# Chanuk-Yang/Deep_Continuous_Fusion_for_Multi-Sensor_3D_Object_Detection

Hardware: AMD Instinct MI355X
Metric: frames/sec (train step) 100k-pt LiDAR + 1242x375 RGB (higher is better)
Workload: dtype bf16; 1 GPU; cfg2: grid 32x704x800, 100000 pts/frame, 1242x375 RGB, ResNet-18 image stream, K=3 fusion x4 sites, eval-mode BN (reference F4), batch 2/GPU; global_batch=2, parallelism=dp1, loss_sampling=compat, conv_chain=False

## Files before the change

### deep_continuous_fusion_for_multi-sensor_3d_object_detection_amd/csrc/conv_common.h

```cpp
#pragma once
#include "dcf_common.h"

namespace {

typedef __bf16 bf16x8 __attribute__((ext_vector_type(8)));
typedef float f32x16 __attribute__((ext_vector_type(16)));
typedef short s16x4 __attribute__((ext_vector_type(4)));

template <int N> __device__ __forceinline__ void wait_vmcnt() { asm volatile("s_waitcnt vmcnt(%0)" ::"n"(N) : "memory"); }
template <int N> __device__ __forceinline__ void wait_vmcnt_nomem() { asm volatile("s_waitcnt vmcnt(%0)" ::"n"(N)); }

__device__ __forceinline__ void glds16(__amdgpu_buffer_rsrc_t rsrc, unsigned voff, unsigned lds_dst)
{
    unsigned keep;
    asm volatile("s_mov_b32 %0, m0\n\ts_mov_b32 m0, %3\n\ts_nop 0\n\tbuffer_load_dwordx4 %1, %2, 0 offen lds\n\ts_mov_b32 m0, %0"
                 : "=&s"(keep)
                 : "v"(voff), "s"(rsrc), "s"(lds_dst)
                 : "memory");
}
__device__ __forceinline__ unsigned lds_addr(const void *p)
{
    return (unsigned)(uintptr_t)(__attribute__((address_space(3))) const char *)p;
}

template <typename V> __device__ __forceinline__ V opaque(V v) { asm volatile("" : "+v"(v)); return v; }

template <typename T> struct Mma;
template <> struct Mma<bf16_t> {
    __device__ static __forceinline__ void run(const uint4 &a, const uint4 &b, f32x16 &acc)
    {
        acc = __builtin_amdgcn_mfma_f32_32x32x16_bf16(__builtin_bit_cast(bf16x8, a), __builtin_bit_cast(bf16x8, b), acc, 0, 0, 0);
    }
};
typedef _Float16 f16x8 __attribute__((ext_vector_type(8)));
template <> struct Mma<f16_t> {
    __device__ static __forceinline__ void run(const uint4 &a, const uint4 &b, f32x16 &acc)
    {
        acc = __builtin_amdgcn_mfma_f32_32x32x16_f16(__builtin_bit_cast(f16x8, a), __builtin_bit_cast(f16x8, b), acc, 0, 0, 0);
    }
};
template <> struct Mma<float> {
// ... 85 lines not shown
```

### deep_continuous_fusion_for_multi-sensor_3d_object_detection_amd/csrc/conv_rs.hip

```cpp
#include "conv_rs_kernel.h"

int dcf_conv3x3_rs_launch(int dtype, const void *x, const void *w, const float *shift, const void *res, const void *mask, void *y,
                          int B, int H, int W, int Ck, int Cn, int relu, int flip, const char *name_base, double flops, hipStream_t s)
{
    if (dtype == DCF_F32 || Ck % 64 || Cn % 64) return DCF_EUNSUPPORTED;
    const int64_t Q = (int64_t)B * H * (W + 2);
    if (Q >= (1ll << 30) || (int64_t)B * H * W * Ck * 2 >= (1ll << 31) || (int64_t)B * H * W * Cn * 2 >= 0xFFFFFF00ll) return DCF_EUNSUPPORTED;
    const RsPlan p = rs_plan(Q, Cn);
    if (p.kind < 0) return DCF_EUNSUPPORTED;
    RsArgs a;
    a.x = (const char *)x; a.w = (const char *)w; a.shift = shift; a.res = (const char *)res; a.mask = (const char *)mask; a.y = (char *)y;
    a.B = B; a.H = H; a.W = W; a.Ck = Ck; a.Cn = Cn; a.relu = relu; a.flip = flip;
    a.npt = p.npt; a.Q = (int)Q;
    a.dbg = dcf_ablate_opt("RS_DBG");
    a.mtiles = (int)((Q + 32 * p.npt - 1) / (32 * p.npt));
    a.xbytes = (unsigned)((int64_t)B * H * W * Ck * 2);
    a.wbytes = (unsigned)((int64_t)Cn * 9 * Ck * 2);
    a.ybytes = (unsigned)((int64_t)B * H * W * Cn * 2);
    const int BN = RS_KINDS[p.kind].BN;
    static DcfOpt pe_o("RS_PERSIST"); const char *pe = pe_o.str();
    int64_t nwg = (((int64_t)a.mtiles * (Cn / BN) + 7) / 8) * 8;
    if (!(pe && atoi(pe) == 0)) nwg = std::min<int64_t>(nwg, 256 * RS_KINDS[p.kind].per_cu);
    const dim3 grid((unsigned)nwg);
    char name[96];
    static DcfOpt pfn_o("RS_PF"); const char *pfn = pfn_o.str();
    static DcfOpt pfn2_o("RS_PF2"), pfl_o("RS_L16"), pfs_o("RS_S3");
    const bool small_pf = p.kind == 2 && !(pfn && atoi(pfn) == 0) && !(pfn2_o.str() && atoi(pfn2_o.str()) == 0) && !(pfl_o.str() && atoi(pfl_o.str()) == 0) &&
                          !(pfs_o.str() && atoi(pfs_o.str()) == 0);
    const bool one_round_n = (Q + 32 * p.npt - 1) / (32 * p.npt) * (Cn / RS_KINDS[p.kind].BN) <= 256 * RS_KINDS[p.kind].per_cu;
    const bool pf_name = small_pf || (p.kind != 2 && ((pfn && atoi(pfn) == 2) || (!(pfn && atoi(pfn) == 0) && (Ck >= 128 || one_round_n))));
    snprintf(name, sizeof(name), pf_name ? "%s<rs%d,%d,pf>" : "%s<rs%d,%d>", name_base, p.kind, p.npt);
    const double bytes = (double)a.xbytes + (double)a.wbytes + (double)B * H * W * Cn * 2.0 * (1 + (res ? 1 : 0) + (mask ? 1 : 0));
    static DcfOpt s3e_o("RS_S3"); const char *s3e = s3e_o.str();
    const bool s3 = !(s3e && atoi(s3e) == 0);
    static DcfOpt l16_o("RS_L16"); const char *l16e = l16_o.str();
    const bool l16 = !(l16e && atoi(l16e) == 0);
    static DcfOpt dx2_o("RS_DX2"); const char *dx2e = dx2_o.str();
    const bool dx2 = p.kind == 1 && p.npt <= 8 && !(dx2e && atoi(dx2e) == 0);
    static DcfOpt pf_o("RS_PF"); const char *pfe = pf_o.str();
    const bool one_round = (int64_t)a.mtiles * (Cn / RS_KINDS[p.kind].BN) <= 256 * RS_KINDS[p.kind].per_cu;
    const bool pf = (pfe && atoi(pfe) == 2) || (!(pfe && atoi(pfe) == 0) && (Ck >= 128 || one_round));
    static DcfOpt pf2_o("RS_PF2"); const char *pf2e = pf2_o.str();
    const bool pf2 = p.kind == 2 && !(pfe && atoi(pfe) == 0) && !(pf2e && atoi(pf2e) == 0);
#define DCF_RS(T_)                                                                                                               \
    do {                                                                                                                         \
        if (p.kind == 0 && pf) DCF_LAUNCH_WB(name, flops, bytes, s, hipLaunchKernelGGL((k_conv3x3_rs<T_, 1, 5, 4, 2, 2, 1, false, false, 0, true>), grid, dim3(512), 0, s, a)); \
        else if (dx2 && pf) DCF_LAUNCH_WB(name, flops, bytes, s, hipLaunchKernelGGL((k_conv3x3_rs<T_, 1, 2, 2, 4, 2, 2, false, false, 0, true>), grid, dim3(512), 0, s, a)); \
        else if (p.kind == 1 && pf) DCF_LAUNCH_WB(name, flops, bytes, s, hipLaunchKernelGGL((k_conv3x3_rs<T_, 1, 3, 2, 4, 2, 1, false, false, 0, true>), grid, dim3(512), 0, s, a)); \
        else if (p.kind == 0) DCF_LAUNCH_WB(name, flops, bytes, s, hipLaunchKernelGGL((k_conv3x3_rs<T_, 1, 5, 4, 2, 2, 1>), grid, dim3(512), 0, s, a)); \
        else if (dx2) DCF_LAUNCH_WB(name, flops, bytes, s, hipLaunchKernelGGL((k_conv3x3_rs<T_, 1, 2, 2, 4, 2, 2>), grid, dim3(512), 0, s, a)); \
        else if (p.kind == 1) DCF_LAUNCH_WB(name, flops, bytes, s, hipLaunchKernelGGL((k_conv3x3_rs<T_, 1, 3, 2, 4, 2, 1>), grid, dim3(512), 0, s, a)); \
        else if (!s3) DCF_LAUNCH_WB(name, flops, bytes, s, hipLaunchKernelGGL((k_conv3x3_rs<T_, 1, 1, 2, 4, 5, 2>), grid, dim3(512), 0, s, a)); \
        else if (l16 && pf2) DCF_LAUNCH_WB(name, flops, bytes, s, hipLaunchKernelGGL((k_conv3x3_rs<T_, 1, 1, 2, 4, 6, 2, true, false, 8, true>), grid, dim3(1024), 0, s, a)); \
        else if (l16) DCF_LAUNCH_WB(name, flops, bytes, s, hipLaunchKernelGGL((k_conv3x3_rs<T_, 1, 1, 2, 4, 6, 2, true, false, 8>), grid, dim3(1024), 0, s, a)); \
        else DCF_LAUNCH_WB(name, flops, bytes, s, hipLaunchKernelGGL((k_conv3x3_rs<T_, 1, 1, 2, 4, 6, 2, true>), grid, dim3(512), 0, s, a)); \
    } while (0)
#ifdef RS_BF16_ONLY
    if (dtype == DCF_F16) return DCF_EUNSUPPORTED;
    DCF_RS(bf16_t);
#else
    if (dtype == DCF_F16) DCF_RS(f16_t); else DCF_RS(bf16_t);
#endif
#undef DCF_RS
    return DCF_OK;
}


#ifdef RS_WSTAMP
extern "C" int dcf_rs_wstamps_read(void *dst, int *dims)
{
    dims[0] = RS_WS_WGS; dims[1] = 8; dims[2] = 3; dims[3] = 64;
    return hipMemcpyFromSymbol(dst, HIP_SYMBOL(g_rs_wstamps), sizeof(g_rs_wstamps)) == hipSuccess ? 0 : -1;
}
extern "C" int dcf_rs_wstamps_clear()
{
    static unsigned zero[RS_WS_WGS * 8 * 3 * 64];
    return hipMemcpyToSymbol(HIP_SYMBOL(g_rs_wstamps), zero, sizeof(zero)) == hipSuccess ? 0 : -1;
}
#endif
```

### deep_continuous_fusion_for_multi-sensor_3d_object_detection_amd/csrc/conv_rs_kernel.h

```cpp
#pragma once
#include <stddef.h>
#include <stdlib.h>

#include <algorithm>
#include <type_traits>

#include "dcf_common.h"
#include "conv_common.h"

#ifndef DCF_RS_SPREAD
#define DCF_RS_SPREAD 1
#endif

namespace {

struct RsArgs {
    const char *x;
    const char *w;
    const float *shift;
    const char *res;
    const char *mask;
    char *y;
    int B, H, W, Ck, Cn;
    int relu, flip;
// ... 1 lines not shown
    int mtiles;
    int Q;
    unsigned xbytes, wbytes, ybytes;
    int dbg;
};

#ifdef RS_STAMP
#define RS_STAMP_WGS 256
#define RS_STAMP_ITEMS 32
__device__ long long g_rs_stamps[RS_STAMP_WGS][RS_STAMP_ITEMS][10];
#define RS_T(k) do { if constexpr (CHAIN) { if (wid == 0) stamp[k] = __builtin_amdgcn_s_memtime(); } } while (0)
#else
#define RS_T(k) do { } while (0)
#endif
#ifdef RS_WSTAMP
#define RS_WS_WGS 256
__device__ unsigned g_rs_wstamps[RS_WS_WGS][8][3][64];
#define RS_WS(reg, idx) do { if constexpr (!CHAIN) { const unsigned t__ = (unsigned)__builtin_amdgcn_s_memtime(); const int i__ = __builtin_amdgcn_readfirstlane(idx); \
    unsigned k__; asm volatile("s_mov_b32 %1, m0\n\ts_mov_b32 m0, %3\n\ts_nop 0\n\tv_writelane_b32 %0, %2, m0\n\ts_mov_b32 m0, %1" : "+v"(reg), "=&s"(k__) : "s"(t__), "s"(i__)); } } while (0)
#else
#define RS_WS(reg, idx) do { } while (0)
#endif
#define RS_CHAIN_MAX 24
struct RsChainLayer {
    const char *x, *w;
    const float *shift;
    const char *res, *mask;
    char *y;
    int relu, pad_;
};
struct RsChainArgs {
    RsArgs a;
    int nlayers;
    int spin_limit;
    int acquire;
    int pad_;
    int *ws;
    RsChainLayer L[RS_CHAIN_MAX];
};
template <typename P> __device__ __forceinline__ P rs_uniform(P p)
{
    const unsigned long long v = (unsigned long long)p;
    const unsigned lo = __builtin_amdgcn_readfirstlane((unsigned)v), hi = __builtin_amdgcn_readfirstlane((unsigned)(v >> 32));
    return (P)(((unsigned long long)hi << 32) | lo);
}
__device__ __forceinline__ const RsArgs &rs_common(const RsArgs &a) { return a; }
// ... 46 lines not shown
    case 5: wait_vmcnt<5>(); break;
    case 6: wait_vmcnt<6>(); break;
    case 7: wait_vmcnt<7>(); break;
    case 8: wait_vmcnt<8>(); break;
    case 9: wait_vmcnt<9>(); break;
    case 10: wait_vmcnt<10>(); break;
    case 11: wait_vmcnt<11>(); break;
    default: wait_vmcnt<12>(); break;
    }
}

constexpr int rs_allowed(int kj, int dw, int dx, int pww, int pxa, int pxb)
{
    int back = dw;
    if (kj == 0 && 3 * dx - 1 < back) back = 3 * dx - 1;
    int n = 0;
    for (int d = 1; d < back; ++d) {
        const int k = ((kj - d) % 3 + 3) % 3;
        n += pww + (k == 0 ? pxa : (k == 1 ? pxb : 0));
    }
    return n;
}

template <typename T, int TN, int TMMAX, int WN, int WM, int DW, int DX, bool S3 = false, bool CHAIN = false, int NL = 0, bool PF = false>
__global__ void __launch_bounds__((WN * WM + NL) * 64) k_conv3x3_rs(typename std::conditional<CHAIN, RsChainArgs, RsArgs>::type arg)
{
    constexpr bool L16 = NL > 0;
    static_assert(!PF || !CHAIN, "the rotated loop: single-layer launches");
    static_assert(!(PF && S3) || NL > 0, "the rotated loop with stage-granular synchronisation: the consumer + loader form only");
    static_assert(!(L16 && CHAIN) && (NL == 0 || NL == 4 || NL == 8), "loader waves: none, four or eight; no chain mode with them");
    const RsArgs &a = rs_common(arg);
    static_assert(DT<T>::size == 2, "16-bit element types only");
    constexpr int NW = WN * WM;
    constexpr int BN = WN * TN * 32;
    constexpr int BMMAX = WM * TMMAX * 32;
    constexpr int NWD = NL ? NL : NW;
    constexpr int PWW = BN / 8 / NWD;
    static_assert(PWW >= 1 && PWW * 8 * NWD == BN, "weight tile must split evenly over the issuing waves");
    constexpr int PXW = (BMMAX + 2 + 8 * NWD - 1) / (8 * NWD);
    constexpr int XROWS = NWD * PXW * 8;
    constexpr int WSLOT = BN * 128, XSLOT = XROWS * 128;
    constexpr int NSW = S3 ? DW + 3 : DW + 1, NSX = DX + 1;
    static_assert(DW >= 1 && DX >= 1 && (DW - 1) * PWW + 2 * PXW <= 48, "vmcnt range");
    static_assert(!S3 || DW == 3 * DX, "stage-granular sync: weights and pixels run the same number of stages ahead");
    static_assert(NSW * WSLOT + NSX * XSLOT <= 160 * 1024, "LDS");
    __shared__ __attribute__((aligned(1024))) char lds[NSW * WSLOT + NSX * XSLOT];

    const int tid = threadIdx.x, lane = tid & 63;
    const int wid16 = __builtin_amdgcn_readfirstlane(tid >> 6);
    const bool loader = L16 && wid16 >= WN * WM;
    const int wid = L16 ? (wid16 >= WN * WM ? wid16 - WN * WM : wid16) : wid16;
    const int wn = wid / WM;
    const int wm = (wid & 4) ? WM - 1 - wid % WM : wid % WM;
    const int r = lane & 31, h = lane >> 5;

    const int nt = a.Cn / BN;
    const int nblk = a.mtiles * nt;
    const int chunk = (nblk + 7) >> 3;
    const int wpx = gridDim.x >> 3;
    const int chunk_lo = (blockIdx.x & 7) * chunk, chunk_hi = min(chunk_lo + chunk, nblk);
    const int gidx_first = chunk_lo + (blockIdx.x >> 3);
    int gidx = gidx_first;
    auto chain_finish = [&]() __attribute__((always_inline)) {
        if constexpr (CHAIN) {
            __builtin_amdgcn_s_barrier();
            int *flag = reinterpret_cast<int *>(lds);
            if (tid == 0) *flag = __hip_atomic_fetch_add(arg.ws, 1, __ATOMIC_RELAXED, __HIP_MEMORY_SCOPE_AGENT) == (int)gridDim.x - 1;
            __syncthreads();
            if (*flag) {
// ... 36 lines not shown
            const kconst_t kp = (kconst_t)__builtin_amdgcn_kernarg_segment_ptr() + offsetof(RsChainArgs, L) +
                                (size_t)__builtin_amdgcn_readfirstlane(l) * sizeof(RsChainLayer);
            const __attribute__((address_space(4))) unsigned long long *q = (const __attribute__((address_space(4))) unsigned long long *)kp;
            static_assert(sizeof(RsChainLayer) == 56 && offsetof(RsChainLayer, y) == 40 && offsetof(RsChainLayer, relu) == 48, "layout read word by word");
            px = (const char *)q[0]; pw = (const char *)q[1]; lshift = (const float *)q[2]; pr = (const char *)q[3]; pm = (const char *)q[4];
            py = (char *)q[5]; lrelu = (int)(unsigned)q[6];
        } else {
            px = a.x; pw = a.w; pr = a.res; pm = a.mask; py = a.y; lshift = a.shift; lrelu = a.relu;
        }
        make_descs();
        res = reinterpret_cast<const T *>(pr);
        mask = reinterpret_cast<const T *>(pm);
    };
    auto bind_weights = [&](int l) __attribute__((always_inline)) {
        if constexpr (CHAIN) {
            typedef const __attribute__((address_space(4))) char *kconst_t;
            const kconst_t kp = (kconst_t)__builtin_amdgcn_kernarg_segment_ptr() + offsetof(RsChainArgs, L) +
                                (size_t)__builtin_amdgcn_readfirstlane(l) * sizeof(RsChainLayer);
            pw = (const char *)((const __attribute__((address_space(4))) unsigned long long *)kp)[1];
            srcW = __builtin_amdgcn_make_buffer_rsrc((void *)rs_uniform(pw), 0, a.wbytes, 0x00020000);
        }
    };
    bind_layer(0);
    constexpr unsigned OOB = 0xFFFFFF00u;
    const unsigned ldsW0 = lds_addr(lds), ldsX0 = ldsW0 + NSW * WSLOT;

    const int l8 = lane >> 3, lc = lane & 7;
    unsigned wbase[PWW];
    const int npieces = (BM + 2 + 7) >> 3;
    const int cntx = __builtin_amdgcn_readfirstlane((L16 && !loader) ? 0 : (wid < npieces ? (npieces - 1 - wid) / NWD + 1 : 0));
    const int pxa = (cntx + 1) >> 1, pxb = cntx >> 1;
    int xbase[PXW], xok[PXW];
    const int rowpitch = a.W * rowbytes;
    auto setup_tile = [&](int gi) __attribute__((always_inline)) {
        n0 = (gi % nt) * BN;
        q0 = (gi / nt) * BM;
#pragma unroll
        for (int j = 0; j < PWW; ++j) {
            const int row = (wid * PWW + j) * 8 + l8;
            wbase[j] = (unsigned)(n0 + row) * (unsigned)(9 * rowbytes) + (unsigned)((lc ^ ((row >> 1) & 7)) * 16);
        }
#pragma unroll
        for (int j = 0; j < PXW; ++j) {
            const int i = (wid + j * NWD) * 8 + l8;
            const int p = q0 - 1 + i;
            const int R = p >= 0 ? p / Wp : 0;
// ... 222 lines not shown
                int wsl = 0, xsl = 0;
                if constexpr (S3) {
#pragma unroll
                    for (int sv = 0; sv < DX; ++sv) {
                        if constexpr (DOX) issue_x(sv, sv, 0, CX);
                        if constexpr (DOW)
#pragma unroll
                            for (int kw = 0; kw < 3; ++kw) issue_w(sv, kw, sv * 3 + kw);
                    }
                } else
#pragma unroll
                for (int u = -3 * DX; u < 0; ++u) {
                    const int v = u + 3 * DX, sv = v / 3, kj = v - 3 * sv;
                    if constexpr (DOX) {
                        if (kj == 0) issue_x(sv, xsl, 0, PXA);
                        if (kj == 1) issue_x(sv, xsl, PXA, CX);
                    }
                    if (kj == 1) ++xsl;
                    if (u + DW >= 0) { if constexpr (DOW) issue_w((u + DW) / 3, (u + DW) % 3, wsl); ++wsl; }
                }
            }
        };
        auto begin_tile = [&]() __attribute__((always_inline)) { begin_tile_parts(std::true_type(), std::true_type()); };
        RS_T(0); RS_T(1);
        begin_tile();
        bool stores_pending = false;
        RS_T(2);
#ifdef RS_WSTAMP
        RS_WS(ws_misc, 1);
#endif
        for (;;) {
        if constexpr (CHAIN) make_descs();
        int wsr = 0, wsi = DW % NSW, xsr = 0, xsi = DX % NSX;
        if constexpr (PF) {
            constexpr int CC = C > 0 ? C : 1;
            uint4 fa0[TN], fb0[CC], fa1[TN], fb1[CC];
            auto load_frags = [&](uint4 (&fa)[TN], uint4 (&fb)[CC], int kj, int ks) __attribute__((always_inline)) {
#if defined(RS_ABL) && (RS_ABL & 2)
                if (kj + ks != 0) return;
#endif
                const char *pw = lds + wsr * WSLOT + rdA;
                const char *px = lds + NSW * WSLOT + xsr * XSLOT + rdX + kj * 128;
                const int swx0 = (h ^ (((r + kj) >> 1) & 7)) << 4;
#pragma unroll
                for (int i = 0; i < TN; ++i) fa[i] = *reinterpret_cast<const uint4 *>(pw + i * 32 * 128 + (swa0 ^ (ks << 5)));
#pragma unroll
// ... 219 lines not shown
                        for (int i = 0; i < TN; ++i) fa[i] = *reinterpret_cast<const uint4 *>(pw + i * 32 * 128 + (swa0 ^ (ks << 5)));
#pragma unroll
                        for (int j = 0; j < C; ++j) fb[j] = *reinterpret_cast<const uint4 *>(px + j * 32 * 128 + (swx0 ^ (ks << 5)));
#pragma unroll
                        for (int j = 0; j < C; ++j)
#pragma unroll
                            for (int i = 0; i < TN; ++i) Mma<T>::run(fa[i], fb[j], acc[i][j]);
                        if (DCF_RS_SPREAD) issue_part(ks);
                    }
                }
                wsr = wsr + 1 == NSW ? 0 : wsr + 1;
                wsi = wsi + 1 == NSW ? 0 : wsi + 1;
            }
            xsr = xsr + 1 == NSX ? 0 : xsr + 1;
            xsi = xsi + 1 == NSX ? 0 : xsi + 1;
#pragma unroll
            for (int d = 0; d < DS; ++d) { wst[d] = wst[d + 1]; xst[d] = xst[d + 1]; kis[d] = kis[d + 1]; }
            stage_entry(DS);
        }
        RS_T(4);
#ifdef RS_WSTAMP
        if (ws_tile == 0) RS_WS(ws_misc, 2);
#endif
        wait_vmcnt<0>();
        RS_T(5);
#ifdef RS_WSTAMP
        if (ws_tile == 0) RS_WS(ws_misc, 3);
#endif
        const int q0c = q0, n0c = n0;
        if constexpr (CHAIN) {
            int ngidx = gidx + wpx, nlayer = layer;
            if (ngidx >= chunk_hi) { nlayer = __builtin_amdgcn_readfirstlane(layer + 1); ngidx = gidx_first; }
            const bool more = nlayer < arg.nlayers;
            if (more) {
                wait_lgkm0();
                __builtin_amdgcn_s_barrier();
                if (nlayer != layer) bind_weights(nlayer);
                if (ngidx != gidx) setup_tile(ngidx);
                begin_tile_parts(std::true_type(), std::false_type());
            }
            store_tile(q0c, n0c);
            RS_T(6);
            wait_vmcnt<0>();
            RS_T(7);
            __builtin_amdgcn_s_barrier();
            if (tid == 0) __hip_atomic_fetch_add(arg.ws + 4 + layer * a.mtiles + q0c / BM, 1, __ATOMIC_RELAXED, __HIP_MEMORY_SCOPE_AGENT);
// ... 11 lines not shown
            if (nlayer != layer) { layer = nlayer; bind_layer(layer); }
            RS_T(0);
            chain_wait();
            RS_T(1);
            begin_tile_parts(std::false_type(), std::true_type());
            RS_T(2);
            wait_vmcnt<0>();
#pragma unroll
            for (int i = 0; i < TN; ++i)
#pragma unroll
                for (int j = 0; j < TMMAX; ++j)
#pragma unroll
                    for (int q = 0; q < 16; ++q) acc[i][j][q] = 0.f;
            continue;
        }
        gidx += wpx;
        const bool more = gidx < chunk_hi;
        if (more) {
            wait_lgkm0();
            __builtin_amdgcn_s_barrier();
            setup_tile(gidx);
            begin_tile();
        }
        store_tile(q0c, n0c);
        stores_pending = true;
#ifdef RS_WSTAMP
        if constexpr (!CHAIN) {
            if (ws_tile == 0) {
                RS_WS(ws_misc, 4);
                if (!more) { wait_vmcnt<0>(); RS_WS(ws_misc, 5); }
            }
            ++ws_tile;
        }
#endif
        if (!more) break;
#pragma unroll
        for (int i = 0; i < TN; ++i)
#pragma unroll
            for (int j = 0; j < TMMAX; ++j)
#pragma unroll
                for (int q = 0; q < 16; ++q) acc[i][j][q] = 0.f;
        }
    };
    if constexpr (L16) {
        if (!loader) {
            switch (cnt) {
            case 0: main_loop(std::integral_constant<int, 0>(), std::integral_constant<int, 0>(), std::true_type()); break;
// ... 81 lines not shown
```

### deep_continuous_fusion_for_multi-sensor_3d_object_detection_amd/csrc/conv_sp.hip

```cpp
#include <stdlib.h>

#include <algorithm>
#include <type_traits>

#include "dcf_common.h"
#include "conv_common.h"

namespace {

struct SpArgs {
    const char *x;
    const char *w;
    const float *shift;
    const char *res;
    const char *mask;
    char *y;
    int B, H, W;
    int relu, flip;
    int txn, tyn;
    int ntiles;
    unsigned xbytes;
    int dbg;
};

typedef unsigned sp_u32x4 __attribute__((ext_vector_type(4)));

template <typename T, int C, int TH, int NBUF>
__global__ void __launch_bounds__(256) __attribute__((amdgpu_waves_per_eu(NBUF == 2 ? 3 : 2, NBUF == 2 ? 3 : 2))) k_conv3x3_sp(SpArgs a)
{
    static_assert(DT<T>::size == 2, "16-bit element types only");
    static_assert(C == 32 || C == 64, "32 or 64 channels");
    constexpr int TW = 32;
    constexpr int PW = C == 64 ? 34 : 36;
    constexpr int RB = C * 2;
    constexpr int NPX = (TH + 2) * PW;
    constexpr int PPP = 1024 / RB;
    constexpr int NPIECE = (NPX + PPP - 1) / PPP;
    constexpr int PXW = (NPIECE + 3) / 4;
    constexpr int WN = C / 32, WM = 4 / WN, TM = TH / WM;
    constexpr int KS = C / 16;
    constexpr int NST = TM * 2;
    static_assert(TH % WM == 0 && (PW * RB) % 256 == 0, "rows must split evenly over the waves; row pitch");
    constexpr int DUMP = NBUF * NPIECE;
    constexpr int AHEAD = (NBUF - 2) * (PXW + NST) + NST;
    static_assert(NBUF >= 2 && AHEAD < 64, "vmcnt range");
    static_assert((NBUF * NPIECE + 1) * 1024 * (NBUF == 2 ? 3 : 2) <= 160 * 1024, "LDS: two workgroups per CU (three with a two-slot ring)");
    __shared__ __attribute__((aligned(1024))) char lds[(NBUF * NPIECE + 1) * 1024];

    const int tid = threadIdx.x, lane = tid & 63;
    const int wid = __builtin_amdgcn_readfirstlane(tid >> 6);
    const int wn = wid % WN, wm = wid / WN;
    const int r = lane & 31, h = lane >> 5;

    const int chunk = (a.ntiles + 7) >> 3;
    const int wpx = gridDim.x >> 3;
    const int chunk_lo = (blockIdx.x & 7) * chunk, chunk_hi = min(chunk_lo + chunk, a.ntiles);
    int t = chunk_lo + (blockIdx.x >> 3);
    if (t >= chunk_hi) return;

    const __amdgpu_buffer_rsrc_t srcX = __builtin_amdgcn_make_buffer_rsrc((void *)a.x, 0, a.xbytes, 0x00020000);
    const __amdgpu_buffer_rsrc_t dstY = __builtin_amdgcn_make_buffer_rsrc((void *)a.y, 0, a.xbytes, 0x00020000);
    constexpr unsigned OOB = 0xFFFFFF00u;
    const unsigned lds0 = lds_addr(lds);

    uint4 wreg[9 * KS];
    {
        const char *wp = a.w + (size_t)(wn * 32 + r) * (9 * RB) + h * 16;
#pragma unroll
        for (int tp = 0; tp < 9; ++tp) {
            const int ts = a.flip ? 8 - tp : tp;
#pragma unroll
            for (int ks = 0; ks < KS; ++ks) wreg[tp * KS + ks] = *reinterpret_cast<const uint4 *>(wp + ts * RB + ks * 32);
        }
    }

    constexpr int CPP = RB / 16;
    auto colkey = [](int cc) { return C == 64 ? (cc >> 1) & 7 : (cc >> 2) & 3; };
    int relo[PXW];
#pragma unroll
    for (int j = 0; j < PXW; ++j) {
        const int p = wid + 4 * j;
        const int i = p * PPP + lane / CPP;
        const int rr_ = i / PW, cc_ = i - rr_ * PW;
        relo[j] = (p < NPIECE && i < NPX) ? (rr_ * a.W + cc_) * RB + (((lane % CPP) ^ colkey(cc_)) << 4) : -1;
// ... 15 lines not shown
            const int ln = opaque(lane);
#pragma unroll
            for (int j = 0; j < PXW; ++j) {
                const int p = wid + 4 * j;
                const int i = p * PPP + ln / CPP;
                const int rr_ = i / PW, cc_ = i - rr_ * PW;
                const int yy = y0 + rr_, xx = x0 + cc_;
                const bool live = tile < chunk_hi && relo[j] >= 0 && yy >= 0 && yy < a.H && xx >= 0 && xx < a.W;
                glds16(srcX, (live && !(DCF_DBG(a) & 2)) ? (unsigned)(org + relo[j]) : OOB,
                       __builtin_amdgcn_readfirstlane(lds0 + (p < NPIECE ? buf * NPIECE + p : DUMP) * 1024));
            }
        }
    };

    int xoff[3][KS];
#pragma unroll
    for (int kj = 0; kj < 3; ++kj)
#pragma unroll
        for (int ks = 0; ks < KS; ++ks) xoff[kj][ks] = (r + kj) * RB + (((2 * ks + h) ^ colkey(r + kj)) << 4);

    const T *res = reinterpret_cast<const T *>(a.res);
    const T *mask = reinterpret_cast<const T *>(a.mask);
    const int c0 = wn * 32 + 8 * h;

#pragma unroll
    for (int d = 0; d < NBUF - 1; ++d) {
        issue_tile(t + d * wpx, d);
#pragma unroll
        for (int k = 0; k < NST; ++k) {
            const sp_u32x4 z = {0u, 0u, 0u, 0u};
            asm volatile("buffer_store_dwordx4 %0, %1, %2, 0 offen\n\ts_nop 1" ::"v"(z), "v"(OOB), "s"(dstY) : "memory");
        }
    }
    int buf = 0;
    for (;;) {
        const int tx = t % a.txn, tq = t / a.txn;
        const int ty = tq % a.tyn, b = tq / a.tyn;
        const int tn = t + wpx;
        wait_vmcnt<AHEAD>();
        __builtin_amdgcn_s_barrier();
        issue_tile(t + (NBUF - 1) * wpx, buf == 0 ? NBUF - 1 : buf - 1);
        const char *tile = lds + buf * (NPIECE * 1024) + wm * TM * PW * RB;
        f32x16 acc[TM];
#pragma unroll
        for (int j = 0; j < TM; ++j)
#pragma unroll
            for (int q = 0; q < 16; ++q) acc[j][q] = 0.f;
        if (!(DCF_DBG(a) & 1))
#pragma unroll
        for (int ki = 0; ki < 3; ++ki)
#pragma unroll
            for (int kj = 0; kj < 3; ++kj) {
                asm volatile("" ::: "memory");
#pragma unroll
                for (int ks = 0; ks < KS; ++ks) {
                    uint4 fb[TM];
#pragma unroll
                    for (int j = 0; j < TM; ++j) fb[j] = *reinterpret_cast<const uint4 *>(tile + xoff[kj][ks] + (j + ki) * PW * RB);
#pragma unroll
                    for (int j = 0; j < TM; ++j) Mma<T>::run(wreg[(ki * 3 + kj) * KS + ks], fb[j], acc[j]);
                }
            }
        int m[TM];
#pragma unroll
        for (int j = 0; j < TM; ++j) {
            const int yy = ty * TH + wm * TM + j, xx = tx * TW + r;
            m[j] = (yy < a.H && xx < a.W) ? (b * a.H + yy) * a.W + xx : -1;
            acc_rows8(acc[j]);
        }
        if (res) {
            uint4 rr[TM][2];
#pragma unroll
            for (int j = 0; j < TM; ++j)
#pragma unroll
                for (int p = 0; p < 2; ++p)
                    rr[j][p] = m[j] >= 0 ? *reinterpret_cast<const uint4 *>(res + (size_t)m[j] * C + c0 + 16 * p) : make_uint4(0, 0, 0, 0);
#pragma unroll
            for (int j = 0; j < TM; ++j)
#pragma unroll
                for (int p = 0; p < 2; ++p) {
                    const unsigned rw[4] = {rr[j][p].x, rr[j][p].y, rr[j][p].z, rr[j][p].w};
#pragma unroll
                    for (int e = 0; e < 4; ++e) {
                        float lo, hi;
                        unpack2<T>(rw[e], lo, hi);
// ... 64 lines not shown
        buf = buf + 1 == NBUF ? 0 : buf + 1;
    }
}

}

int dcf_conv3x3_sp_launch(int dtype, const void *x, const void *w, const float *shift, const void *res, const void *mask, void *y,
                          int B, int H, int W, int Ck, int Cn, int relu, int flip, const char *name_base, double flops, hipStream_t s)
{
    static DcfOpt on_o("CONV_SP"), minpix_o("CONV_SP_MIN_PIX"), wgpc_o("CONV_SP_WGPC");
    const char *on = on_o.str(), *mp = minpix_o.str(), *wg = wgpc_o.str();
    if (on && atoi(on) == 0) return DCF_EUNSUPPORTED;
    if (dtype == DCF_F32 || Ck != Cn || (Ck != 32 && Ck != 64)) return DCF_EUNSUPPORTED;
    const int64_t npix = (int64_t)B * H * W;
    if (npix < (mp ? atoll(mp) : 200000ll) || npix * Ck * 2 >= (1ll << 31)) return DCF_EUNSUPPORTED;
    const int TH = Ck == 32 ? 8 : 4;
    SpArgs a;
    a.x = (const char *)x; a.w = (const char *)w; a.shift = shift; a.res = (const char *)res; a.mask = (const char *)mask; a.y = (char *)y;
    a.B = B; a.H = H; a.W = W; a.relu = relu; a.flip = flip;
    a.txn = (W + 31) / 32; a.tyn = (H + TH - 1) / TH;
    a.ntiles = B * a.txn * a.tyn;
    a.xbytes = (unsigned)(npix * Ck * 2);
    a.dbg = dcf_ablate_opt("SP_DBG");
    static DcfOpt nb_o("CONV_SP_NBUF32");
    const char *nb = nb_o.str();
    const bool ring2 = Ck == 32 && !(nb && atoi(nb) == 3);
    const int wgpc = wg ? atoi(wg) : (ring2 ? 3 : 2);
    const int64_t nwg = std::min<int64_t>(((int64_t)a.ntiles + 7) / 8 * 8, 256 * wgpc);
    const dim3 grid((unsigned)nwg);
    char name[96];
    snprintf(name, sizeof(name), "%s<sp%d>", name_base, Ck);
    const double bytes = (double)npix * Ck * 2.0 * (2 + (res ? 1 : 0) + (mask ? 1 : 0)) + 9.0 * Ck * Cn * 2.0;
#define DCF_SP(T_)                                                                                                                \
    do {                                                                                                                          \
        if (Ck == 32 && ring2) DCF_LAUNCH_WB(name, flops, bytes, s, hipLaunchKernelGGL((k_conv3x3_sp<T_, 32, 8, 2>), grid, dim3(256), 0, s, a)); \
        else if (Ck == 32) DCF_LAUNCH_WB(name, flops, bytes, s, hipLaunchKernelGGL((k_conv3x3_sp<T_, 32, 8, 3>), grid, dim3(256), 0, s, a)); \
        else DCF_LAUNCH_WB(name, flops, bytes, s, hipLaunchKernelGGL((k_conv3x3_sp<T_, 64, 4, 3>), grid, dim3(256), 0, s, a));       \
    } while (0)
    if (dtype == DCF_F16) DCF_SP(f16_t); else DCF_SP(bf16_t);
#undef DCF_SP
    return DCF_OK;
}
```

Baseline: 382.9 frames/s.

## Prefetch residual/mask epilogue operands and stage BN shift in LDS for conv kernels

Adds a new epilogue path to the RS and SP 3x3 conv kernels. Residual and mask tiles are issued as async buffer loads early, before or during the MMA loop, and waited on with counted vmcnt. The per-channel shift is cached in LDS. Stores go through buffer stores with OOB masking. This hides the global-load latency of the epilogue behind compute, at the cost of extra VGPRs for in-flight operands, more LDS, and more complex vmcnt bookkeeping. Kind-0 RS launches and Cn above 1024 fall back to the old path through a second compiled copy of the launcher.

```diff
diff --git a/deep_continuous_fusion_for_multi-sensor_3d_object_detection_amd/csrc/conv_common.h b/deep_continuous_fusion_for_multi-sensor_3d_object_detection_amd/csrc/conv_common.h
--- a/deep_continuous_fusion_for_multi-sensor_3d_object_detection_amd/csrc/conv_common.h
+++ b/deep_continuous_fusion_for_multi-sensor_3d_object_detection_amd/csrc/conv_common.h
@@ -17,6 +17,18 @@
                  : "=&s"(keep)
                  : "v"(voff), "s"(rsrc), "s"(lds_dst)
                  : "memory");
+}
+typedef unsigned epi_u32x4 __attribute__((ext_vector_type(4)));
+template <int IMM = 0, bool SC1 = false> __device__ __forceinline__ void gld16(epi_u32x4 &d, __amdgpu_buffer_rsrc_t rsrc, unsigned voff)
+{
+    if constexpr (SC1) asm volatile("buffer_load_dwordx4 %0, %1, %2, 0 offen offset:%3 sc1" : "=v"(d) : "v"(voff), "s"(rsrc), "n"(IMM) : "memory");
+    else asm volatile("buffer_load_dwordx4 %0, %1, %2, 0 offen offset:%3" : "=v"(d) : "v"(voff), "s"(rsrc), "n"(IMM) : "memory");
+}
+__device__ __forceinline__ void epi_bind(epi_u32x4 &v) { asm volatile("" : "+v"(v)); }
+template <int BASE, int STEP> __device__ __forceinline__ void wait_vmcnt_k(int k)
+{
+    static_assert(BASE + 2 * STEP < 64, "vmcnt range");
+    if (k == 0) wait_vmcnt<BASE>(); else if (k == 1) wait_vmcnt<BASE + STEP>(); else wait_vmcnt<BASE + 2 * STEP>();
 }
 __device__ __forceinline__ unsigned lds_addr(const void *p)
 {
diff --git a/deep_continuous_fusion_for_multi-sensor_3d_object_detection_amd/csrc/conv_rs.hip b/deep_continuous_fusion_for_multi-sensor_3d_object_detection_amd/csrc/conv_rs.hip
--- a/deep_continuous_fusion_for_multi-sensor_3d_object_detection_amd/csrc/conv_rs.hip
+++ b/deep_continuous_fusion_for_multi-sensor_3d_object_detection_amd/csrc/conv_rs.hip
@@ -1,13 +1,33 @@
 #include "conv_rs_kernel.h"
 
+#ifndef RS_EPI_FORM
+#define RS_EPI_FORM 1
+#endif
+
+int dcf_conv3x3_rs_launch_epi0(int dtype, const void *x, const void *w, const float *shift, const void *res, const void *mask, void *y,
+                               int B, int H, int W, int Ck, int Cn, int relu, int flip, const char *name_base, double flops, hipStream_t s);
+
+#if RS_EPI_FORM
 int dcf_conv3x3_rs_launch(int dtype, const void *x, const void *w, const float *shift, const void *res, const void *mask, void *y,
                           int B, int H, int W, int Ck, int Cn, int relu, int flip, const char *name_base, double flops, hipStream_t s)
+#else
+int dcf_conv3x3_rs_launch_epi0(int dtype, const void *x, const void *w, const float *shift, const void *res, const void *mask, void *y,
+                               int B, int H, int W, int Ck, int Cn, int relu, int flip, const char *name_base, double flops, hipStream_t s)
+#endif
 {
+#if RS_EPI_FORM
+    static DcfOpt epi_o("CONV_EPI");
+    if ((epi_o.str() && atoi(epi_o.str()) == 0) || Cn > RS_EPI_MAXCN) return dcf_conv3x3_rs_launch_epi0(dtype, x, w, shift, res, mask, y, B, H, W, Ck, Cn, relu, flip, name_base, flops, s);
+#endif
+    constexpr bool E = RS_EPI_FORM != 0;
     if (dtype == DCF_F32 || Ck % 64 || Cn % 64) return DCF_EUNSUPPORTED;
     const int64_t Q = (int64_t)B * H * (W + 2);
     if (Q >= (1ll << 30) || (int64_t)B * H * W * Ck * 2 >= (1ll << 31) || (int64_t)B * H * W * Cn * 2 >= 0xFFFFFF00ll) return DCF_EUNSUPPORTED;
     const RsPlan p = rs_plan(Q, Cn);
     if (p.kind < 0) return DCF_EUNSUPPORTED;
+#if RS_EPI_FORM
+    if (p.kind == 0) return dcf_conv3x3_rs_launch_epi0(dtype, x, w, shift, res, mask, y, B, H, W, Ck, Cn, relu, flip, name_base, flops, s);
+#endif
     RsArgs a;
     a.x = (const char *)x; a.w = (const char *)w; a.shift = shift; a.res = (const char *)res; a.mask = (const char *)mask; a.y = (char *)y;
     a.B = B; a.H = H; a.W = W; a.Ck = Ck; a.Cn = Cn; a.relu = relu; a.flip = flip;
@@ -42,18 +62,24 @@
     const bool pf = (pfe && atoi(pfe) == 2) || (!(pfe && atoi(pfe) == 0) && (Ck >= 128 || one_round));
     static DcfOpt pf2_o("RS_PF2"); const char *pf2e = pf2_o.str();
     const bool pf2 = p.kind == 2 && !(pfe && atoi(pfe) == 0) && !(pf2e && atoi(pf2e) == 0);
+#if RS_EPI_FORM
+#define DCF_RS_K0(T_) if (false) { }
+#else
+#define DCF_RS_K0(T_)                                                                                                            \
+        if (p.kind == 0 && pf) DCF_LAUNCH_WB(name, flops, bytes, s, hipLaunchKernelGGL((k_conv3x3_rs<T_, 1, 5, 4, 2, 2, 1, false, false, 0, true, E>), grid, dim3(512), 0, s, a)); \
+        else if (p.kind == 0) DCF_LAUNCH_WB(name, flops, bytes, s, hipLaunchKernelGGL((k_conv3x3_rs<T_, 1, 5, 4, 2, 2, 1, false, false, 0, false, E>), grid, dim3(512), 0, s, a));
+#endif
 #define DCF_RS(T_)                                                                                                               \
     do {                                                                                                                         \
-        if (p.kind == 0 && pf) DCF_LAUNCH_WB(name, flops, bytes, s, hipLaunchKernelGGL((k_conv3x3_rs<T_, 1, 5, 4, 2, 2, 1, false, false, 0, true>), grid, dim3(512), 0, s, a)); \
-        else if (dx2 && pf) DCF_LAUNCH_WB(name, flops, bytes, s, hipLaunchKernelGGL((k_conv3x3_rs<T_, 1, 2, 2, 4, 2, 2, false, false, 0, true>), grid, dim3(512), 0, s, a)); \
-        else if (p.kind == 1 && pf) DCF_LAUNCH_WB(name, flops, bytes, s, hipLaunchKernelGGL((k_conv3x3_rs<T_, 1, 3, 2, 4, 2, 1, false, false, 0, true>), grid, dim3(512), 0, s, a)); \
-        else if (p.kind == 0) DCF_LAUNCH_WB(name, flops, bytes, s, hipLaunchKernelGGL((k_conv3x3_rs<T_, 1, 5, 4, 2, 2, 1>), grid, dim3(512), 0, s, a)); \
-        else if (dx2) DCF_LAUNCH_WB(name, flops, bytes, s, hipLaunchKernelGGL((k_conv3x3_rs<T_, 1, 2, 2, 4, 2, 2>), grid, dim3(512), 0, s, a)); \
-        else if (p.kind == 1) DCF_LAUNCH_WB(name, flops, bytes, s, hipLaunchKernelGGL((k_conv3x3_rs<T_, 1, 3, 2, 4, 2, 1>), grid, dim3(512), 0, s, a)); \
-        else if (!s3) DCF_LAUNCH_WB(name, flops, bytes, s, hipLaunchKernelGGL((k_conv3x3_rs<T_, 1, 1, 2, 4, 5, 2>), grid, dim3(512), 0, s, a)); \
-        else if (l16 && pf2) DCF_LAUNCH_WB(name, flops, bytes, s, hipLaunchKernelGGL((k_conv3x3_rs<T_, 1, 1, 2, 4, 6, 2, true, false, 8, true>), grid, dim3(1024), 0, s, a)); \
-        else if (l16) DCF_LAUNCH_WB(name, flops, bytes, s, hipLaunchKernelGGL((k_conv3x3_rs<T_, 1, 1, 2, 4, 6, 2, true, false, 8>), grid, dim3(1024), 0, s, a)); \
-        else DCF_LAUNCH_WB(name, flops, bytes, s, hipLaunchKernelGGL((k_conv3x3_rs<T_, 1, 1, 2, 4, 6, 2, true>), grid, dim3(512), 0, s, a)); \
+        DCF_RS_K0(T_)                                                                                                            \
+        else if (dx2 && pf) DCF_LAUNCH_WB(name, flops, bytes, s, hipLaunchKernelGGL((k_conv3x3_rs<T_, 1, 2, 2, 4, 2, 2, false, false, 0, true, E>), grid, dim3(512), 0, s, a)); \
+        else if (p.kind == 1 && pf) DCF_LAUNCH_WB(name, flops, bytes, s, hipLaunchKernelGGL((k_conv3x3_rs<T_, 1, 3, 2, 4, 2, 1, false, false, 0, true, E>), grid, dim3(512), 0, s, a)); \
+        else if (dx2) DCF_LAUNCH_WB(name, flops, bytes, s, hipLaunchKernelGGL((k_conv3x3_rs<T_, 1, 2, 2, 4, 2, 2, false, false, 0, false, E>), grid, dim3(512), 0, s, a)); \
+        else if (p.kind == 1) DCF_LAUNCH_WB(name, flops, bytes, s, hipLaunchKernelGGL((k_conv3x3_rs<T_, 1, 3, 2, 4, 2, 1, false, false, 0, false, E>), grid, dim3(512), 0, s, a)); \
+        else if (!s3) DCF_LAUNCH_WB(name, flops, bytes, s, hipLaunchKernelGGL((k_conv3x3_rs<T_, 1, 1, 2, 4, 5, 2, false, false, 0, false, E>), grid, dim3(512), 0, s, a)); \
+        else if (l16 && pf2) DCF_LAUNCH_WB(name, flops, bytes, s, hipLaunchKernelGGL((k_conv3x3_rs<T_, 1, 1, 2, 4, 6, 2, true, false, 8, true, E>), grid, dim3(1024), 0, s, a)); \
+        else if (l16) DCF_LAUNCH_WB(name, flops, bytes, s, hipLaunchKernelGGL((k_conv3x3_rs<T_, 1, 1, 2, 4, 6, 2, true, false, 8, false, E>), grid, dim3(1024), 0, s, a)); \
+        else DCF_LAUNCH_WB(name, flops, bytes, s, hipLaunchKernelGGL((k_conv3x3_rs<T_, 1, 1, 2, 4, 6, 2, true, false, 0, false, E>), grid, dim3(512), 0, s, a)); \
     } while (0)
 #ifdef RS_BF16_ONLY
     if (dtype == DCF_F16) return DCF_EUNSUPPORTED;
@@ -62,11 +88,12 @@
     if (dtype == DCF_F16) DCF_RS(f16_t); else DCF_RS(bf16_t);
 #endif
 #undef DCF_RS
+#undef DCF_RS_K0
     return DCF_OK;
 }
 
 
-#ifdef RS_WSTAMP
+#if defined(RS_WSTAMP) && RS_EPI_FORM
 extern "C" int dcf_rs_wstamps_read(void *dst, int *dims)
 {
     dims[0] = RS_WS_WGS; dims[1] = 8; dims[2] = 3; dims[3] = 64;
diff --git a/deep_continuous_fusion_for_multi-sensor_3d_object_detection_amd/csrc/conv_rs_kernel.h b/deep_continuous_fusion_for_multi-sensor_3d_object_detection_amd/csrc/conv_rs_kernel.h
--- a/deep_continuous_fusion_for_multi-sensor_3d_object_detection_amd/csrc/conv_rs_kernel.h
+++ b/deep_continuous_fusion_for_multi-sensor_3d_object_detection_amd/csrc/conv_rs_kernel.h
@@ -47,6 +47,7 @@
 #define RS_WS(reg, idx) do { } while (0)
 #endif
 #define RS_CHAIN_MAX 24
+#define RS_EPI_MAXCN 1024
 struct RsChainLayer {
     const char *x, *w;
     const float *shift;
@@ -139,11 +140,12 @@
     return n;
 }
 
-template <typename T, int TN, int TMMAX, int WN, int WM, int DW, int DX, bool S3 = false, bool CHAIN = false, int NL = 0, bool PF = false>
+template <typename T, int TN, int TMMAX, int WN, int WM, int DW, int DX, bool S3 = false, bool CHAIN = false, int NL = 0, bool PF = false, bool EPI = false>
 __global__ void __launch_bounds__((WN * WM + NL) * 64) k_conv3x3_rs(typename std::conditional<CHAIN, RsChainArgs, RsArgs>::type arg)
 {
     constexpr bool L16 = NL > 0;
     static_assert(!PF || !CHAIN, "the rotated loop: single-layer launches");
+    static_assert(!EPI || !CHAIN, "the one-round epilogue: single-layer launches (chain residuals are sc1 hand-off loads)");
     static_assert(!(PF && S3) || NL > 0, "the rotated loop with stage-granular synchronisation: the consumer + loader form only");
     static_assert(!(L16 && CHAIN) && (NL == 0 || NL == 4 || NL == 8), "loader waves: none, four or eight; no chain mode with them");
     const RsArgs &a = rs_common(arg);
@@ -160,8 +162,9 @@
     constexpr int NSW = S3 ? DW + 3 : DW + 1, NSX = DX + 1;
     static_assert(DW >= 1 && DX >= 1 && (DW - 1) * PWW + 2 * PXW <= 48, "vmcnt range");
     static_assert(!S3 || DW == 3 * DX, "stage-granular sync: weights and pixels run the same number of stages ahead");
-    static_assert(NSW * WSLOT + NSX * XSLOT <= 160 * 1024, "LDS");
-    __shared__ __attribute__((aligned(1024))) char lds[NSW * WSLOT + NSX * XSLOT];
+    constexpr int LSH = NSW * WSLOT + NSX * XSLOT;
+    static_assert(LSH + (EPI ? RS_EPI_MAXCN * 4 : 0) <= 160 * 1024, "LDS");
+    __shared__ __attribute__((aligned(1024))) char lds[LSH + (EPI ? RS_EPI_MAXCN * 4 : 0)];
 
     const int tid = threadIdx.x, lane = tid & 63;
     const int wid16 = __builtin_amdgcn_readfirstlane(tid >> 6);
@@ -244,6 +247,12 @@
         }
     };
     bind_layer(0);
+    if constexpr (EPI) {
+        if (lshift) {
+            for (int i = tid; i < a.Cn; i += (NW + NL) * 64) reinterpret_cast<float *>(lds + LSH)[i] = lshift[i];
+            wait_lgkm0();
+        }
+    }
     constexpr unsigned OOB = 0xFFFFFF00u;
     const unsigned ldsW0 = lds_addr(lds), ldsX0 = ldsW0 + NSW * WSLOT;
 
@@ -512,6 +521,114 @@
             }
         };
         auto begin_tile = [&]() __attribute__((always_inline)) { begin_tile_parts(std::true_type(), std::true_type()); };
+        constexpr bool BOTH = TMMAX <= 2;
+        constexpr int CE = C > 0 ? C : 1;
+        constexpr int NR = C * TN * 2;
+        constexpr int NPRO = NI ? 0 : (S3 ? DX * (CX + 3 * PWW) : DX * CX + (DW < 3 * DX ? DW : 3 * DX) * PWW);
+        static_assert(2 * NR < 64, "vmcnt range");
+        auto issue_op = [&](const char *src, const unsigned (&eo)[CE], epi_u32x4 (&e)[CE][TN][2]) __attribute__((always_inline)) {
+            const __amdgpu_buffer_rsrc_t rs = __builtin_amdgcn_make_buffer_rsrc((void *)src, 0, a.ybytes, 0x00020000);
+#pragma unroll
+            for (int j = 0; j < C; ++j)
+#pragma unroll
+                for (int i = 0; i < TN; ++i) {
+                    const unsigned o = (i == 0 || eo[j] == OOB) ? eo[j] : eo[j] + (unsigned)(i * 64);
+                    gld16<0>(e[j][i][0], rs, o); gld16<32>(e[j][i][1], rs, o);
+                }
+        };
+        auto epi_issue = [&](int q0c, int n0c, unsigned (&eo)[CE], epi_u32x4 (&e1)[CE][TN][2], epi_u32x4 (&e2)[BOTH ? CE : 1][TN][2]) __attribute__((always_inline)) {
+#pragma unroll
+            for (int j = 0; j < C; ++j) {
+                const int p = q0c + (pt0 + j) * 32 + r;
+                const int R = p / Wp, c = p - R * Wp;
+                const bool valid = !(p >= a.Q || c < 1 || c > a.W);
+                eo[j] = valid ? (unsigned)((R * a.W + c - 1) * a.Cn + n0c + wn * TN * 32 + 8 * h) * 2u : OOB;
+            }
+            if (res || mask) issue_op(res ? (const char *)res : (const char *)mask, eo, e1);
+            if constexpr (BOTH) { if (res && mask) issue_op((const char *)mask, eo, e2); }
+        };
+        auto use_res = [&](epi_u32x4 (&e)[CE][TN][2]) __attribute__((always_inline)) {
+#pragma unroll
+            for (int j = 0; j < C; ++j)
+#pragma unroll
+                for (int i = 0; i < TN; ++i)
+#pragma unroll
+                    for (int pp = 0; pp < 2; ++pp) {
+                        epi_bind(e[j][i][pp]);
+#pragma unroll
+                        for (int k = 0; k < 4; ++k) {
+                            float lo, hi;
+                            unpack2<T>(e[j][i][pp][k], lo, hi);
+                            acc[i][j][8 * pp + 2 * k] += lo; acc[i][j][8 * pp + 2 * k + 1] += hi;
+                        }
+                    }
+        };
+        auto use_mask = [&](epi_u32x4 (&e)[CE][TN][2]) __attribute__((always_inline)) {
+#pragma unroll
+            for (int j = 0; j < C; ++j)
+#pragma unroll
+                for (int i = 0; i < TN; ++i)
+#pragma unroll
+                    for (int pp = 0; pp < 2; ++pp) {
+                        epi_bind(e[j][i][pp]);
+#pragma unroll
+                        for (int k = 0; k < 4; ++k) {
+                            float lo, hi;
+                            unpack2<T>(e[j][i][pp][k], lo, hi);
+                            if (!(lo > 0.f)) acc[i][j][8 * pp + 2 * k] = 0.f;
+                            if (!(hi > 0.f)) acc[i][j][8 * pp + 2 * k + 1] = 0.f;
+                        }
+                    }
+        };
+        auto epi_store = [&](bool pieces_behind, int n0c, const unsigned (&eo)[CE], epi_u32x4 (&e1)[CE][TN][2], epi_u32x4 (&e2)[BOTH ? CE : 1][TN][2]) __attribute__((always_inline)) {
+#pragma unroll
+            for (int i = 0; i < TN; ++i)
+#pragma unroll
+                for (int j = 0; j < C; ++j) acc_rows8(acc[i][j]);
+            if (res || mask) { if (pieces_behind) wait_vmcnt<(NPRO < 63 ? NPRO : 63)>(); else wait_vmcnt<0>(); }
+            if (res) use_res(e1);
+            const bool late_m = !BOTH && res && mask;
+            if (late_m) issue_op((const char *)mask, eo, e1);
+            if (lshift) {
+                const float *ls = reinterpret_cast<const float *>(lds + LSH) + n0c + wn * TN * 32 + 8 * h;
+#pragma unroll
+                for (int i = 0; i < TN; ++i)
+#pragma unroll
+                    for (int pp = 0; pp < 2; ++pp) {
+                        float sh[8];
+#pragma unroll
+                        for (int k = 0; k < 8; ++k) sh[k] = ls[i * 32 + 16 * pp + k];
+#pragma unroll
+                        for (int j = 0; j < C; ++j)
+#pragma unroll
+                            for (int k = 0; k < 8; ++k) acc[i][j][8 * pp + k] += sh[k];
+                    }
+            }
+            if (lrelu) {
+#pragma unroll
+                for (int i = 0; i < TN; ++i)
+#pragma unroll
+                    for (int j = 0; j < C; ++j)
+#pragma unroll
+                        for (int k = 0; k < 16; ++k) acc[i][j][k] = fmaxf(acc[i][j][k], 0.f);
+            }
+            if (mask) {
+                if (late_m) wait_vmcnt<0>();
+                if constexpr (BOTH) { if (res) use_mask(e2); else use_mask(e1); }
+                else use_mask(e1);
+            }
+#pragma unroll
+            for (int j = 0; j < C; ++j)
+#pragma unroll
+                for (int i = 0; i < TN; ++i)
+#pragma unroll
+                    for (int pp = 0; pp < 2; ++pp) {
+                        float v[8];
+#pragma unroll
+                        for (int k = 0; k < 8; ++k) v[k] = acc[i][j][8 * pp + k];
+                        gst16<0>(dstY, eo[j] == OOB ? OOB : eo[j] + (unsigned)(i * 64 + pp * 32), pack8<T>(v));
+                    }
+        };
         RS_T(0); RS_T(1);
         begin_tile();
         bool stores_pending = false;
@@ -777,6 +894,13 @@
 #ifdef RS_WSTAMP
         if (ws_tile == 0) RS_WS(ws_misc, 2);
 #endif
+        const bool enew = EPI && C > 0 && !(DCF_DBG(a) & 4);
+        unsigned eo[CE];
+        epi_u32x4 e1[CE][TN][2], e2[BOTH ? CE : 1][TN][2];
+        if (enew) {
+            epi_issue(q0, n0, eo, e1, e2);
+            wait_vmcnt_k<0, NR>(!(res || mask) ? 0 : (BOTH && res && mask) ? 2 : 1);
+        } else
         wait_vmcnt<0>();
         RS_T(5);
 #ifdef RS_WSTAMP
@@ -834,7 +958,7 @@
             setup_tile(gidx);
             begin_tile();
         }
-        store_tile(q0c, n0c);
+        if (enew) epi_store(more, n0c, eo, e1, e2); else store_tile(q0c, n0c);
         stores_pending = true;
 #ifdef RS_WSTAMP
         if constexpr (!CHAIN) {
diff --git a/deep_continuous_fusion_for_multi-sensor_3d_object_detection_amd/csrc/conv_sp.hip b/deep_continuous_fusion_for_multi-sensor_3d_object_detection_amd/csrc/conv_sp.hip
--- a/deep_continuous_fusion_for_multi-sensor_3d_object_detection_amd/csrc/conv_sp.hip
+++ b/deep_continuous_fusion_for_multi-sensor_3d_object_detection_amd/csrc/conv_sp.hip
@@ -25,7 +25,7 @@
 
 typedef unsigned sp_u32x4 __attribute__((ext_vector_type(4)));
 
-template <typename T, int C, int TH, int NBUF>
+template <typename T, int C, int TH, int NBUF, bool EPI>
 __global__ void __launch_bounds__(256) __attribute__((amdgpu_waves_per_eu(NBUF == 2 ? 3 : 2, NBUF == 2 ? 3 : 2))) k_conv3x3_sp(SpArgs a)
 {
     static_assert(DT<T>::size == 2, "16-bit element types only");
@@ -44,8 +44,12 @@
     constexpr int DUMP = NBUF * NPIECE;
     constexpr int AHEAD = (NBUF - 2) * (PXW + NST) + NST;
     static_assert(NBUF >= 2 && AHEAD < 64, "vmcnt range");
-    static_assert((NBUF * NPIECE + 1) * 1024 * (NBUF == 2 ? 3 : 2) <= 160 * 1024, "LDS: two workgroups per CU (three with a two-slot ring)");
-    __shared__ __attribute__((aligned(1024))) char lds[(NBUF * NPIECE + 1) * 1024];
+    constexpr int NE = TM * 2;
+    constexpr int ES = (NBUF == 2 || C == 64) ? 0 : 2;
+    constexpr int LSH = (NBUF * NPIECE + 1) * 1024;
+    static_assert(AHEAD + (NBUF - 2) * 2 * NE < 64 && PXW + NE < 64, "vmcnt range");
+    static_assert((LSH + C * 4) * (NBUF == 2 ? 3 : 2) <= 160 * 1024, "LDS: two workgroups per CU (three with a two-slot ring)");
+    __shared__ __attribute__((aligned(1024))) char lds[LSH + C * 4];
 
     const int tid = threadIdx.x, lane = tid & 63;
     const int wid = __builtin_amdgcn_readfirstlane(tid >> 6);
@@ -60,6 +64,8 @@
 
     const __amdgpu_buffer_rsrc_t srcX = __builtin_amdgcn_make_buffer_rsrc((void *)a.x, 0, a.xbytes, 0x00020000);
     const __amdgpu_buffer_rsrc_t dstY = __builtin_amdgcn_make_buffer_rsrc((void *)a.y, 0, a.xbytes, 0x00020000);
+    const __amdgpu_buffer_rsrc_t srcR = __builtin_amdgcn_make_buffer_rsrc((void *)(a.res ? a.res : a.y), 0, a.xbytes, 0x00020000);
+    const __amdgpu_buffer_rsrc_t srcM = __builtin_amdgcn_make_buffer_rsrc((void *)(a.mask ? a.mask : a.y), 0, a.xbytes, 0x00020000);
     constexpr unsigned OOB = 0xFFFFFF00u;
     const unsigned lds0 = lds_addr(lds);
 
@@ -121,12 +127,65 @@
     const T *res = reinterpret_cast<const T *>(a.res);
     const T *mask = reinterpret_cast<const T *>(a.mask);
     const int c0 = wn * 32 + 8 * h;
+    constexpr bool epi = EPI;
+    const bool has_r = res != nullptr, has_m = mask != nullptr;
+    const int ke = (!epi || ES == 0) ? 0 : ES == 2 ? (has_r ? 1 : 0) + (has_m ? 1 : 0) : ((has_r || has_m) ? 1 : 0);
+    const bool late_r = epi && ES == 0 && has_r;
+    const bool late_m = epi && has_m && (ES == 0 || (ES == 1 && has_r));
+    const float *lsh = reinterpret_cast<const float *>(lds + LSH);
+    if (epi && a.shift) {
+        if (tid < C) reinterpret_cast<float *>(lds + LSH)[tid] = a.shift[tid];
+        asm volatile("s_waitcnt lgkmcnt(0)" ::: "memory");
+    }
+    auto issue_epi = [&](const unsigned (&eo)[TM], epi_u32x4 (&e1)[TM][2], epi_u32x4 (&e2)[TM][2]) __attribute__((always_inline)) {
+        if (ke == 0) return;
+        if (has_r) {
+#pragma unroll
+            for (int j = 0; j < TM; ++j) { gld16<0>(e1[j][0], srcR, eo[j]); gld16<32>(e1[j][1], srcR, eo[j]); }
+        }
+        if (has_m && (ES == 2 || !has_r)) {
+#pragma unroll
+            for (int j = 0; j < TM; ++j) {
+                if constexpr (ES == 2) { gld16<0>(e2[j][0], srcM, eo[j]); gld16<32>(e2[j][1], srcM, eo[j]); }
+                else { gld16<0>(e1[j][0], srcM, eo[j]); gld16<32>(e1[j][1], srcM, eo[j]); }
+            }
+        }
+    };
+    auto add_res = [&](f32x16 (&acc)[TM], epi_u32x4 (&e)[TM][2]) __attribute__((always_inline)) {
+#pragma unroll
+        for (int j = 0; j < TM; ++j)
+#pragma unroll
+            for (int p = 0; p < 2; ++p) {
+                epi_bind(e[j][p]);
+#pragma unroll
+                for (int q = 0; q < 4; ++q) {
+                    float lo, hi;
+                    unpack2<T>(e[j][p][q], lo, hi);
+                    acc[j][8 * p + 2 * q] += lo; acc[j][8 * p + 2 * q + 1] += hi;
+                }
+            }
+    };
+    auto apply_mask = [&](f32x16 (&acc)[TM], epi_u32x4 (&e)[TM][2]) __attribute__((always_inline)) {
+#pragma unroll
+        for (int j = 0; j < TM; ++j)
+#pragma unroll
+            for (int p = 0; p < 2; ++p) {
+                epi_bind(e[j][p]);
+#pragma unroll
+                for (int q = 0; q < 4; ++q) {
+                    float lo, hi;
+                    unpack2<T>(e[j][p][q], lo, hi);
+                    if (!(lo > 0.f)) acc[j][8 * p + 2 * q] = 0.f;
+                    if (!(hi > 0.f)) acc[j][8 * p + 2 * q + 1] = 0.f;
+                }
+            }
+    };
 
 #pragma unroll
     for (int d = 0; d < NBUF - 1; ++d) {
         issue_tile(t + d * wpx, d);
 #pragma unroll
-        for (int k = 0; k < NST; ++k) {
+        for (int k = 0; k < NST + (d + 1 < NBUF - 1 ? ke * NE : 0); ++k) {
             const sp_u32x4 z = {0u, 0u, 0u, 0u};
             asm volatile("buffer_store_dwordx4 %0, %1, %2, 0 offen\n\ts_nop 1" ::"v"(z), "v"(OOB), "s"(dstY) : "memory");
         }
@@ -136,8 +195,18 @@
         const int tx = t % a.txn, tq = t / a.txn;
         const int ty = tq % a.tyn, b = tq / a.tyn;
         const int tn = t + wpx;
-        wait_vmcnt<AHEAD>();
+        wait_vmcnt_k<AHEAD, (NBUF - 2) * NE>(ke);
         __builtin_amdgcn_s_barrier();
+        unsigned eo[TM];
+        epi_u32x4 e1[TM][2], e2[TM][2];
+        auto tile_offsets = [&]() __attribute__((always_inline)) {
+#pragma unroll
+            for (int j = 0; j < TM; ++j) {
+                const int yy = ty * TH + wm * TM + j, xx = tx * TW + r;
+                eo[j] = (yy < a.H && xx < a.W) ? (unsigned)(((b * a.H + yy) * a.W + xx) * C + c0) * 2u : OOB;
+            }
+        };
+        if (epi && ES > 0) { tile_offsets(); issue_epi(eo, e1, e2); }
         issue_tile(t + (NBUF - 1) * wpx, buf == 0 ? NBUF - 1 : buf - 1);
         const char *tile = lds + buf * (NPIECE * 1024) + wm * TM * PW * RB;
         f32x16 acc[TM];
@@ -160,6 +229,72 @@
                     for (int j = 0; j < TM; ++j) Mma<T>::run(wreg[(ki * 3 + kj) * KS + ks], fb[j], acc[j]);
                 }
             }
+        if (epi) {
+            if (ES == 0) tile_offsets();
+#pragma unroll
+            for (int j = 0; j < TM; ++j) acc_rows8(acc[j]);
+            if (late_r) {
+#pragma unroll
+                for (int j = 0; j < TM; ++j) { gld16<0>(e1[j][0], srcR, eo[j]); gld16<32>(e1[j][1], srcR, eo[j]); }
+            }
+            if (has_r) {
+                if constexpr (ES == 2) wait_vmcnt_k<PXW, NE>(has_m ? 1 : 0); else if constexpr (ES == 1) wait_vmcnt<PXW>(); else wait_vmcnt<0>();
+                add_res(acc, e1);
+            }
+            if (late_m) {
+#pragma unroll
+                for (int j = 0; j < TM; ++j) { gld16<0>(e2[j][0], srcM, eo[j]); gld16<32>(e2[j][1], srcM, eo[j]); }
+            }
+            if (a.shift) {
+#pragma unroll
+                for (int p = 0; p < 2; ++p) {
+                    float sh[8];
+#pragma unroll
+                    for (int k = 0; k < 8; ++k) sh[k] = lsh[c0 + 16 * p + k];
+#pragma unroll
+                    for (int j = 0; j < TM; ++j)
+#pragma unroll
+                        for (int k = 0; k < 8; ++k) acc[j][8 * p + k] += sh[k];
+                }
+            }
+            if (a.relu) {
+#pragma unroll
+                for (int j = 0; j < TM; ++j)
+#pragma unroll
+                    for (int k = 0; k < 16; ++k) acc[j][k] = fmaxf(acc[j][k], 0.f);
+            }
+            if (has_m) {
+                if (late_m) { wait_vmcnt<0>(); apply_mask(acc, e2); }
+                else {
+                    wait_vmcnt<PXW>();
+                    if constexpr (ES == 2) apply_mask(acc, e2); else apply_mask(acc, e1);
+                }
+            }
+#pragma unroll
+            for (int j = 0; j < TM; ++j)
+#pragma unroll
+                for (int p = 0; p < 2; ++p) {
+                    float v[8];
+#pragma unroll
+                    for (int k = 0; k < 8; ++k) v[k] = acc[j][8 * p + k];
+                    uint4 pk;
+                    if constexpr (std::is_same<T, bf16_t>::value) {
+                        pk = make_uint4(pack2bf(v[0], v[1]), pack2bf(v[2], v[3]), pack2bf(v[4], v[5]), pack2bf(v[6], v[7]));
+                    } else {
+                        typedef _Float16 h16x8 __attribute__((ext_vector_type(8)));
+                        h16x8 hv;
+#pragma unroll
+                        for (int k = 0; k < 8; ++k) hv[k] = (_Float16)v[k];
+                        pk = __builtin_bit_cast(uint4, hv);
+                    }
+                    const sp_u32x4 d = {pk.x, pk.y, pk.z, pk.w};
+                    __builtin_amdgcn_raw_buffer_store_b128(d, dstY, (eo[j] != OOB && !(DCF_DBG(a) & 4)) ? (int)(eo[j] + 32u * p) : (int)OOB, 0, 0);
+                }
+            if (tn >= chunk_hi) break;
+            t = tn;
+            buf = buf + 1 == NBUF ? 0 : buf + 1;
+            continue;
+        }
         int m[TM];
 #pragma unroll
         for (int j = 0; j < TM; ++j) {
@@ -270,6 +405,8 @@
     a.ntiles = B * a.txn * a.tyn;
     a.xbytes = (unsigned)(npix * Ck * 2);
     a.dbg = dcf_ablate_opt("SP_DBG");
+    static DcfOpt epi_o("CONV_EPI");
+    const bool epi = !(epi_o.str() && atoi(epi_o.str()) == 0);
     static DcfOpt nb_o("CONV_SP_NBUF32");
     const char *nb = nb_o.str();
     const bool ring2 = Ck == 32 && !(nb && atoi(nb) == 3);
@@ -279,13 +416,14 @@
     char name[96];
     snprintf(name, sizeof(name), "%s<sp%d>", name_base, Ck);
     const double bytes = (double)npix * Ck * 2.0 * (2 + (res ? 1 : 0) + (mask ? 1 : 0)) + 9.0 * Ck * Cn * 2.0;
-#define DCF_SP(T_)                                                                                                                \
+#define DCF_SP(T_, E_)                                                                                                            \
     do {                                                                                                                          \
-        if (Ck == 32 && ring2) DCF_LAUNCH_WB(name, flops, bytes, s, hipLaunchKernelGGL((k_conv3x3_sp<T_, 32, 8, 2>), grid, dim3(256), 0, s, a)); \
-        else if (Ck == 32) DCF_LAUNCH_WB(name, flops, bytes, s, hipLaunchKernelGGL((k_conv3x3_sp<T_, 32, 8, 3>), grid, dim3(256), 0, s, a)); \
-        else DCF_LAUNCH_WB(name, flops, bytes, s, hipLaunchKernelGGL((k_conv3x3_sp<T_, 64, 4, 3>), grid, dim3(256), 0, s, a));       \
+        if (Ck == 32 && ring2) DCF_LAUNCH_WB(name, flops, bytes, s, hipLaunchKernelGGL((k_conv3x3_sp<T_, 32, 8, 2, E_>), grid, dim3(256), 0, s, a)); \
+        else if (Ck == 32) DCF_LAUNCH_WB(name, flops, bytes, s, hipLaunchKernelGGL((k_conv3x3_sp<T_, 32, 8, 3, E_>), grid, dim3(256), 0, s, a)); \
+        else DCF_LAUNCH_WB(name, flops, bytes, s, hipLaunchKernelGGL((k_conv3x3_sp<T_, 64, 4, 3, E_>), grid, dim3(256), 0, s, a));   \
     } while (0)
-    if (dtype == DCF_F16) DCF_SP(f16_t); else DCF_SP(bf16_t);
+    if (dtype == DCF_F16) { if (epi) DCF_SP(f16_t, true); else DCF_SP(f16_t, false); }
+    else { if (epi) DCF_SP(bf16_t, true); else DCF_SP(bf16_t, false); }
 #undef DCF_SP
     return DCF_OK;
 }
```

Result: no change. 382.9 frames/s (median of 3 runs) (-0.0%).
